# facebookresearch/nonrigid_nerf

Hardware: NVIDIA H100
Metric: rays/sec (64c+128f samples, 8x256 MLP), example_sequence training step (higher is better)
Workload: dtype f16 (tensor-core operands; f32 accumulate)

## Files before the change

### include/nrnerf_b200.h

```cpp
#ifndef NRNERF_B200_H
#define NRNERF_B200_H

#include <stddef.h>
#include <stdint.h>

#ifdef __cplusplus
extern "C" {
#endif

#define NRN_ABI_VERSION 4

#define NRN_OK 0
#define NRN_E_INVALID (-1)
#define NRN_E_CUDA (-2)
#define NRN_E_DEVICE (-3)

int nrn_abi_version(void);
const char* nrn_last_error(void);

int nrn_device_error(int* code_out);

size_t nrn_packed_nerf_bytes(void);
size_t nrn_packed_bender_bytes(void);
int nrn_pack_nerf(const float* const* w, const float* const* b, int input_ch, int out_ch, void* packed,
// ... 69 lines not shown
  const float* d_acc_map;
  float* d_raw;
  void* stream;
} NrnCompositeBwdArgs;
int nrn_composite_backward(const NrnCompositeBwdArgs* args);

size_t nrn_stash_bytes(int n_rays, int n_samples);
size_t nrn_grad_stash_bytes(int n_rays, int n_samples);
size_t nrn_relu_mask_bytes(int n_rays, int n_samples);
size_t nrn_wgrad_scratch_bytes(void);
int nrn_nerf_grad_floats(int out_ch);
int nrn_bender_grad_floats(void);
typedef struct NrnFieldBwdArgs {
  int32_t n_rays, n_samples, out_ch;
  const float* d_raw;
  const void* stash;
  void* grad_stash;
  float* wgrad_scratch;
  const void* nerf_packed;
  const void* bender_packed;
  const float* unmasked_offsets;
  const float* rigidity_mask;
  const float* d_unmasked_offsets;
  const float* d_rigidity_mask;
  int32_t use_cutoff;  float rigidity_cutoff;
  int32_t use_scaling; float scaling;
  float* nerf_grad;
  float* bender_grad;
  float* d_latents;
  void* stream;
  float* nerf_grad_head;
  int32_t accumulate_nerf, accumulate_bender;
  const void* relu_mask;
} NrnFieldBwdArgs;
int nrn_field_backward(const NrnFieldBwdArgs* args);

int nrn_tc_latent_bias(const float* latents, int64_t latent_stride, int n_rays, const float* w0, const float* b0, const float* w5,
                       const float* b5, float* ray_bias, void* stream);
int nrn_field_forward_tc(const NrnFieldArgs* args, const float* ray_bias);
int nrn_nerf_tc_grad_floats(int out_ch);

size_t nrn_packed_views_bytes(void);
int nrn_pack_views(const float* const* w, const float* const* b, void* packed, void* stream);
size_t nrn_views_workspace_bytes(int n_rays, int n_samples);
typedef struct NrnViewArgs {
  const void* views_packed;
  const float* viewdirs;
  int64_t viewdirs_stride;
  void* workspace;
} NrnViewArgs;
int nrn_field_forward_views(const NrnFieldArgs* args, const NrnViewArgs* views);
size_t nrn_packed_views_t_bytes(void);
int nrn_pack_views_t(const float* const* w, void* packed, void* stream);
size_t nrn_views_stash_bytes(int n_rays, int n_samples);
size_t nrn_views_grad_stash_bytes(int n_rays, int n_samples);
size_t nrn_hv_mask_bytes(int n_rays, int n_samples);
int nrn_nerf_views_grad_floats(void);
typedef struct NrnViewTrainArgs {
  void* views_stash;
  void* hv_mask;
} NrnViewTrainArgs;
int nrn_field_forward_views_train(const NrnFieldArgs* args, const NrnViewArgs* views, const NrnViewTrainArgs* train);
typedef struct NrnViewBwdArgs {
  const void* views_t_packed;
  const void* views_stash;
  void* views_grad_stash;
// ... 159 lines not shown
```

### nonrigid_nerf_b200/_lib.py

```python
from __future__ import annotations

import ctypes as C
import os
import threading

_HERE = os.path.dirname(os.path.abspath(__file__))
LIB_PATH = os.path.join(_HERE, "libnrnerf_b200.so")
ABI_VERSION = 4

_f32p = C.POINTER(C.c_float)
_vp = C.c_void_p


class NrnFieldArgs(C.Structure):
    _fields_ = [
        ("rays", _vp), ("z_vals", _vp), ("points", _vp), ("points_stride", C.c_int64),
        ("latents", _vp), ("latent_stride", C.c_int64),
        ("n_rays", C.c_int32), ("n_samples", C.c_int32),
        ("nerf_packed", _vp), ("bender_packed", _vp),
        ("out_ch", C.c_int32),
        ("use_cutoff", C.c_int32), ("rigidity_cutoff", C.c_float),
        ("use_scaling", C.c_int32), ("scaling", C.c_float),
        ("use_removal", C.c_int32), ("removal_threshold", C.c_float),
        ("raw", _vp), ("initial_input_pts", _vp), ("input_pts", _vp), ("unmasked_offsets", _vp),
        ("masked_offsets", _vp), ("rigidity_mask", _vp),
        ("stash", _vp),
        ("stream", _vp),
        ("relu_mask", _vp),
    ]


class NrnViewArgs(C.Structure):
    _fields_ = [
        ("views_packed", _vp), ("viewdirs", _vp), ("viewdirs_stride", C.c_int64), ("workspace", _vp),
    ]


class NrnViewTrainArgs(C.Structure):
    _fields_ = [("views_stash", _vp), ("hv_mask", _vp)]


class NrnViewBwdArgs(C.Structure):
    _fields_ = [("views_t_packed", _vp), ("views_stash", _vp), ("views_grad_stash", _vp), ("hv_mask", _vp)]


class NrnFieldBwdArgs(C.Structure):
    _fields_ = [
        ("n_rays", C.c_int32), ("n_samples", C.c_int32), ("out_ch", C.c_int32),
        ("d_raw", _vp), ("stash", _vp), ("grad_stash", _vp), ("wgrad_scratch", _vp),
        ("nerf_packed", _vp), ("bender_packed", _vp),
        ("unmasked_offsets", _vp), ("rigidity_mask", _vp), ("d_unmasked_offsets", _vp), ("d_rigidity_mask", _vp),
        ("use_cutoff", C.c_int32), ("rigidity_cutoff", C.c_float),
        ("use_scaling", C.c_int32), ("scaling", C.c_float),
        ("nerf_grad", _vp), ("bender_grad", _vp), ("d_latents", _vp),
        ("stream", _vp),
        ("nerf_grad_head", _vp), ("accumulate_nerf", C.c_int32), ("accumulate_bender", C.c_int32),
        ("relu_mask", _vp),
    ]


class NrnTcBwdArgs(C.Structure):
    _fields_ = [
        ("latents", _vp), ("latent_stride", C.c_int64), ("w0", _vp), ("w5", _vp), ("d_latents", _vp), ("workspace", _vp),
    ]


class NrnDivArgs(C.Structure):
    _fields_ = [
        ("n_rays", C.c_int32), ("n_samples", C.c_int32),
        ("relu_mask", _vp), ("e", _vp), ("unmasked_offsets", _vp), ("rigidity_mask", _vp), ("weights", _vp),
        ("weights_are_opacity_alpha", C.c_int32),
        ("bender_packed", _vp),
        ("tangent_stash", _vp), ("d", _vp), ("alpha", _vp), ("beta", _vp), ("tau_c", _vp), ("loss", _vp),
        ("G", _vp), ("g_ray", _vp), ("G_workspace", _vp), ("adjoint_stash", _vp), ("wgrad_scratch", _vp), ("d_unmasked_offsets", _vp),
        ("d_rigidity_mask", _vp), ("bender_grad", _vp),
        ("stream", _vp),
        ("accumulate_bender", C.c_int32),
    ]


class NrnRayLossArgs(C.Structure):
    _fields_ = [
        ("n_rays", C.c_int32), ("n_samples", C.c_int32),
        ("rgb", _vp), ("rgb0", _vp), ("target", _vp), ("weights", _vp), ("unmasked_offsets", _vp), ("rigidity_mask", _vp),
        ("lam_offsets", C.c_float), ("lam_rigidity", C.c_float),
        ("loss", _vp), ("u_rgb", _vp), ("u_rgb0", _vp), ("u_unmasked_offsets", _vp), ("u_rigidity_mask", _vp),
        ("stream", _vp),
        ("sched_step", _vp), ("sched_n_iters", C.c_float), ("divergence", _vp), ("lam_divergence", C.c_float), ("u_divergence", _vp),
    ]

# ... 195 lines not shown
```

### nonrigid_nerf_b200/autograd.py

```python
from __future__ import annotations

import ctypes as C
from typing import Dict, Optional, Tuple

import torch

from . import _lib, ops


def _knobs(net):
    bender = net.ray_bender[0]
    cutoff = getattr(bender, "rigidity_test_time_cutoff", None) if bender is not None else None
    scaling = getattr(bender, "test_time_scaling", None) if bender is not None else None
    removal = getattr(net, "test_time_nonrigid_object_removal_threshold", None)
    return cutoff, scaling, removal


def _tc_net(net):
    if not getattr(net, "time_conditioned_baseline", False):
        return None
    if net.ray_bender[0] is not None:
        raise RuntimeError("nonrigid_nerf_b200: the time_conditioned_baseline NeRF requires ray bending to be turned off "
                           "(ray_bender must be None)")
    return net
# ... 14 lines not shown
        for i in range(3):
            bend += [rig_w[i], rig_b[i]]
    return nerf, bend


def _split_flat(flat: torch.Tensor, like):
    out, o = [], 0
    for p in like:
        n = p.numel()
        out.append(flat[o:o + n].view_as(p))
        o += n
    assert o == flat.numel(), (o, flat.numel())
    return out


def check_held_out(held_out: Optional[torch.Tensor], n_rays: int, device) -> Optional[torch.Tensor]:
    if held_out is None:
        return None
    if not isinstance(held_out, torch.Tensor):
        raise RuntimeError("nonrigid_nerf_b200: held_out must be a tensor ([N] bool or uint8, one entry per ray)")
    if held_out.dtype not in (torch.bool, torch.uint8):
        raise RuntimeError(f"nonrigid_nerf_b200: held_out must be bool or uint8 (0/1 per ray), got {held_out.dtype}")
    if held_out.dim() != 1 or held_out.shape[0] != n_rays:
        raise RuntimeError(f"nonrigid_nerf_b200: held_out must have shape [{n_rays}] (one entry per ray), got {list(held_out.shape)}")
    if held_out.device != torch.device(device):
        raise RuntimeError(f"nonrigid_nerf_b200: held_out must be on the rays' device {device}, got {held_out.device}")
    return held_out.contiguous().view(torch.uint8)


def _zero_held_rows(d_raw: torch.Tensor, held: Optional[torch.Tensor]) -> torch.Tensor:
    if held is None:
        return d_raw
    return d_raw.masked_fill(held.view(-1, 1, 1).bool(), 0.0)


class _FieldTrainFn(torch.autograd.Function):

    @staticmethod
    def forward(ctx, net, rays, z_vals, latents, held, n_nerf, *params):
        bender = net.ray_bender[0]
        cutoff, scaling, removal = _knobs(net)
        if removal is not None:
            raise RuntimeError("nonrigid_nerf_b200: test_time_nonrigid_object_removal_threshold is a test-time knob; "
                               "it is not differentiable")
        nerf_pack = ops.pack_nerf(net)
        bender_pack = ops.pack_bender(bender) if bender is not None else None
        out_ch = net.output_linear.weight.shape[0]
        n, s = z_vals.shape
        lib = _lib.load()
        stash = torch.empty(lib.nrn_stash_bytes(n, s), dtype=torch.uint8, device=z_vals.device)
        relu_mask = torch.empty(lib.nrn_relu_mask_bytes(n, s), dtype=torch.uint8, device=z_vals.device)
        tc = _tc_net(net)
        ctx.tc_latents = None
        if tc is not None:
            ctx.tc_latents = ops.latent_rows(latents.detach(), n, z_vals.device)
            latents = ctx.tc_latents[0]
        raw, det = ops.field_forward(rays, z_vals, latents, nerf_pack, bender_pack, out_ch, cutoff, scaling, None, True, stash,
                                     relu_mask, tc)
        ctx.net, ctx.n_nerf = net, n_nerf
        ctx.shape = (n, s, out_ch)
        ctx.knobs = (cutoff, scaling)
        ctx.packs = (nerf_pack, bender_pack)
        ctx.stash = stash
        ctx.relu_mask = relu_mask
        ctx.params = params
        ctx.held = held
# ... 40 lines not shown
        nerf_grad, a.nerf_grad, a.nerf_grad_head, a.accumulate_nerf = _grad_destination(nerf_p, len(nerf_p) - 2, n_floats, dev)
        bend_grad = d_lat = None
        keep = [d_raw]
        if bender is not None:
            un, rig = ctx.saved_tensors
            a.bender_packed = bender_pack.data_ptr()
            a.unmasked_offsets, a.rigidity_mask = un.data_ptr(), rig.data_ptr()
            if d_un is not None:
                d_un = d_un.contiguous().float()
                a.d_unmasked_offsets = d_un.data_ptr()
                keep.append(d_un)
            if d_rig is not None:
                d_rig = d_rig.contiguous().float()
                a.d_rigidity_mask = d_rig.data_ptr()
                keep.append(d_rig)
            if cutoff is not None:
                a.use_cutoff, a.rigidity_cutoff = 1, float(cutoff)
            if scaling is not None:
                a.use_scaling, a.scaling = 1, float(scaling)
            bend_p = list(ctx.params[ctx.n_nerf:])
            bend_grad, a.bender_grad, _, a.accumulate_bender = _grad_destination(bend_p, len(bend_p), lib.nrn_bender_grad_floats(), dev)
            d_lat = torch.empty(n, ops.LATENT, dtype=torch.float32, device=dev)
            a.d_latents = d_lat.data_ptr()
        a.stream = torch.cuda.current_stream().cuda_stream
        if ctx.tc_latents is not None:
            lat, stride = ctx.tc_latents
            t = _lib.NrnTcBwdArgs()
            t.latents, t.latent_stride = lat.data_ptr(), stride
            t.w0, t.w5 = net.pts_linears[0].weight.data_ptr(), net.pts_linears[5].weight.data_ptr()
            d_lat = torch.empty(n, ops.LATENT, dtype=torch.float32, device=dev)
            workspace = torch.empty(lib.nrn_tc_workspace_bytes(n), dtype=torch.uint8, device=dev)
            t.d_latents, t.workspace = d_lat.data_ptr(), workspace.data_ptr()
            with torch.cuda.device(dev):
                _lib.check(lib.nrn_field_backward_tc(C.byref(a), C.byref(t)), "field_backward_tc")
        elif bender is not None and torch.are_deterministic_algorithms_enabled():
            rows = torch.empty(lib.nrn_latent_rows_bytes(n, s) // 4, dtype=torch.float32, device=dev)
            with torch.cuda.device(dev):
                if held is not None:
                    _lib.check(lib.nrn_field_backward_det_held_out(C.byref(a), rows.data_ptr(), held.data_ptr()), "field_backward_det_held_out")
                else:
                    _lib.check(lib.nrn_field_backward_det(C.byref(a), rows.data_ptr()), "field_backward_det")
        elif held is not None:
            with torch.cuda.device(dev):
                _lib.check(lib.nrn_field_backward_held_out(C.byref(a), held.data_ptr()), "field_backward_held_out")
        else:
            with torch.cuda.device(dev):
                _lib.check(lib.nrn_field_backward(C.byref(a)), "field_backward")
        grads = _param_grads(nerf_grad, nerf_p)
        if bender is not None:
            grads += _param_grads(bend_grad, bend_p)
        return (None, None, None, d_lat, None, None, *grads)


def _arena_destination(params):
    from .optim import arena_destination
    return arena_destination(list(params))


def _grad_destination(params, split: int, n_floats: int, dev):
    if all(p.requires_grad for p in params):
        dst = _arena_destination(params[:split])
        head = _arena_destination(params[split:]) if dst is not None and split < len(params) else None
        if dst is not None and (head is not None or split == len(params)):
            return None, dst, head, 1
    flat = torch.empty(n_floats, dtype=torch.float32, device=dev)
    return flat, flat.data_ptr(), None, 0


def _param_grads(flat: Optional[torch.Tensor], params):
    if flat is None:
        return [None] * len(params)
    return [g if p.requires_grad else None for g, p in zip(_split_flat(flat, params), params)]


class _LatentGatherFn(torch.autograd.Function):

    @staticmethod
    def forward(ctx, timestep, *latents):
        z = latents[0].numel()
        base, contiguous = latents[0].data_ptr(), True
# ... 85 lines not shown
        ctx.shape = (n, s)
        a = _div_args(ctx)
        a.loss = loss.data_ptr()
        if torch.are_deterministic_algorithms_enabled():
            rows = torch.empty(lib.nrn_div_loss_rows_bytes(n, s) // 4, dtype=torch.float32, device=dev)
            with torch.cuda.device(dev):
                _lib.check(lib.nrn_divergence_forward_det(C.byref(a), rows.data_ptr()), "divergence_forward_det")
        else:
            with torch.cuda.device(dev):
                _lib.check(lib.nrn_divergence_forward(C.byref(a)), "divergence_forward")
        ctx.bend_p = bend_p
        ctx.held = held
        ctx.in_shapes = (unmasked.shape, rigidity.shape)
        return loss

    @staticmethod
    def backward(ctx, g):
        n, s = ctx.shape
        dev = ctx.keep[0].device
        lib = _lib.load()
        g = g.reshape(n).contiguous().float()
        G = torch.empty(n * s, dtype=torch.float32, device=dev)
        a = _div_args(ctx)
        a.g_ray, a.G_workspace = g.data_ptr(), G.data_ptr()
        adj = torch.empty(lib.nrn_div_grad_stash_bytes(n, s), dtype=torch.uint8, device=dev)
        scratch = torch.empty(lib.nrn_wgrad_scratch_bytes(), dtype=torch.uint8, device=dev)
        d_un = torch.empty(n * s, 3, dtype=torch.float32, device=dev)
        d_rg = torch.empty(n * s, dtype=torch.float32, device=dev)
        bend_p = list(ctx.bend_p)
        bend_grad, a.bender_grad, _, a.accumulate_bender = _grad_destination(bend_p, len(bend_p), lib.nrn_bender_grad_floats(), dev)
        a.adjoint_stash, a.wgrad_scratch = adj.data_ptr(), scratch.data_ptr()
        a.d_unmasked_offsets, a.d_rigidity_mask = d_un.data_ptr(), d_rg.data_ptr()
        with torch.cuda.device(dev):
            if ctx.held is not None:
                _lib.check(lib.nrn_divergence_backward_held_out(C.byref(a), ctx.held.data_ptr()), "divergence_backward_held_out")
            else:
                _lib.check(lib.nrn_divergence_backward(C.byref(a)), "divergence_backward")
        return (d_un.view(ctx.in_shapes[0]), d_rg.view(ctx.in_shapes[1]), None, None, None, None, None, None,
                *_param_grads(bend_grad, bend_p))


def divergence_loss(unmasked: torch.Tensor, rigidity: torch.Tensor, weights: Optional[torch.Tensor], bender,
                    e: Optional[torch.Tensor] = None, opacity_alpha: Optional[torch.Tensor] = None,
                    held_out: Optional[torch.Tensor] = None) -> torch.Tensor:
    held = check_held_out(held_out, unmasked.shape[0], unmasked.device)
    relu_mask = lookup_relu_mask(unmasked)
    if relu_mask is None:
        raise RuntimeError("nonrigid_nerf_b200: no ReLU masks for these offsets -- the fused divergence term needs the "
                           "un-chunked coarse pass of the current differentiable render() call (N_rand <= chunk)")
    n, s = unmasked.shape[0], unmasked.shape[1]
    if e is None:
        e = torch.randn(n * s, 3, device=unmasked.device)
    _, bend_p = _flat_params(None, bender)
    if opacity_alpha is not None:
        return _DivergenceFn.apply(unmasked, rigidity, opacity_alpha, e, relu_mask, bender, True, held, *bend_p)
    return _DivergenceFn.apply(unmasked, rigidity, weights, e, relu_mask, bender, False, held, *bend_p)


class _RayLossFn(torch.autograd.Function):

    @staticmethod
    def forward(ctx, rgb, rgb0, target, weights, unmasked, rigidity, lam_o, lam_r, sched_step, sched_n_iters, div, lam_div):
        n = rgb.shape[0]
        dev = rgb.device
        lib = _lib.load()
        a = _lib.NrnRayLossArgs()
# ... 256 lines not shown
```

### nonrigid_nerf_b200/csrc/c_abi.cu

```cuda
#include <cstdarg>
#include <cstdio>
#include <cstring>
#include <cstdlib>
#include "../../include/nrnerf_b200.h"
#include "nrn_common.cuh"
#include "pack.cuh"
#include "ray_ops.cuh"
#include "wgrad.cuh"
#include "div.cuh"
#include "loss.cuh"
#include "adam.cuh"
#include "peer.cuh"
#include "det_reduce.cuh"
#include "eval.cuh"

namespace nrn {
cudaError_t launch_field_fwd(const FieldFwdParams& p, bool has_bender, int num_sms, cudaStream_t stream);
cudaError_t launch_field_bwd(const FieldBwdParams& p, bool has_bender, int num_sms, cudaStream_t stream);
cudaError_t launch_field_bwd_det(const FieldBwdParams& p, float* latent_rows, int num_sms, cudaStream_t stream);
cudaError_t launch_field_bwd_held(const FieldBwdParams& p, float* latent_rows, const uint8_t* held, int num_sms, cudaStream_t stream);
cudaError_t launch_field_fwd_tc(const FieldFwdParams& p, int num_sms, cudaStream_t stream);
cudaError_t launch_tc_latent_bias(const float* lat, long long lat_stride, int n_rays, const float* w0, const float* b0, const float* w5,
                                  const float* b5, float* rb, cudaStream_t stream);
cudaError_t launch_tc_latent_bwd(const TcBwdParams& p, cudaStream_t stream);
cudaError_t launch_field_bend(const FieldFwdParams& p, const ViewParams& v, int num_sms, cudaStream_t stream);
cudaError_t launch_field_views(const FieldFwdParams& p, const ViewParams& v, int num_sms, cudaStream_t stream);
cudaError_t launch_field_views_train(const FieldFwdParams& p, const ViewParams& v, const ViewTrainParams& t, int num_sms, cudaStream_t stream);
cudaError_t launch_field_bwd_views(const FieldBwdParams& p, const ViewBwdParams& v, int num_sms, cudaStream_t stream);
}

namespace {

thread_local char g_err[512] = "";

int fail(int code, const char* fmt, ...) {
  va_list ap;
  va_start(ap, fmt);
  vsnprintf(g_err, sizeof(g_err), fmt, ap);
  va_end(ap);
  return code;
}
int cuda_fail(cudaError_t e, const char* what) {
  return fail(NRN_E_CUDA, "%s: %s", what, cudaGetErrorString(e));
}

constexpr int kMaxDevices = 64;
struct DeviceState {
  int* err_word = nullptr;
  int num_sms = 0;
};
DeviceState g_dev[kMaxDevices];

int device_state(DeviceState** out) {
  int dev = 0;
  cudaError_t e = cudaGetDevice(&dev);
  if (e != cudaSuccess) return cuda_fail(e, "cudaGetDevice");
  if (dev < 0 || dev >= kMaxDevices) return fail(NRN_E_INVALID, "device index %d out of range", dev);
  DeviceState& s = g_dev[dev];
  if (!s.err_word) {
    cudaDeviceProp prop;
    e = cudaGetDeviceProperties(&prop, dev);
    if (e != cudaSuccess) return cuda_fail(e, "cudaGetDeviceProperties");
    if (prop.major != 9 || prop.minor != 0)
      return fail(NRN_E_INVALID, "nrnerf_b200 is built for sm_90a (H100) only, found sm_%d%d", prop.major, prop.minor);
    s.num_sms = prop.multiProcessorCount;
    if (const char* g = getenv("NRN_GRID")) { const int v = atoi(g); if (v > 0 && v < s.num_sms) s.num_sms = v; }
    e = cudaMalloc(&s.err_word, 4 * sizeof(int));
    if (e != cudaSuccess) return cuda_fail(e, "cudaMalloc(err word)");
    e = cudaMemset(s.err_word, 0, 4 * sizeof(int));
    if (e != cudaSuccess) return cuda_fail(e, "cudaMemset(err word)");
  }
  *out = &s;
  return NRN_OK;
}

bool aligned16(const void* p) { return (reinterpret_cast<uintptr_t>(p) & 15u) == 0; }

struct TimedLaunch {
  cudaEvent_t a, b;
  int kind;
};
bool g_timing = false;
// ... 463 lines not shown
  cudaStream_t st = static_cast<cudaStream_t>(a->stream);
  return timed(4, st, "composite_bwd_kernel", [&] { return nrn::launch_composite_bwd(p, st); });
}

size_t nrn_stash_bytes(int n_rays, int n_samples) { return static_cast<size_t>(even_tiles(n_rays, n_samples)) * nrn::kStashTileBytes; }
size_t nrn_grad_stash_bytes(int n_rays, int n_samples) { return static_cast<size_t>(even_tiles(n_rays, n_samples)) * nrn::kGradTileBytes; }
size_t nrn_relu_mask_bytes(int n_rays, int n_samples) { return static_cast<size_t>(even_tiles(n_rays, n_samples)) * nrn::kMaskTileBytes; }
size_t nrn_wgrad_scratch_bytes(void) { return static_cast<size_t>(nrn::kWgMaxCtas) * nrn::kWgScratchFloats * sizeof(float); }
int nrn_nerf_grad_floats(int out_ch) { return nrn::nerf_grad_floats(out_ch); }
int nrn_bender_grad_floats(void) { return nrn::bparam::total(); }
int nrn_nerf_tc_grad_floats(int out_ch) { return nrn::nerf_tc_grad_floats(out_ch); }
size_t nrn_tc_workspace_bytes(int n_rays) { return n_rays < 0 ? 0 : (static_cast<size_t>(n_rays) * 2 * 256 + 2 * 256 * nrn::kLatent) * sizeof(float); }

static int field_backward(const NrnFieldBwdArgs* a, const NrnTcBwdArgs* t, const char* who, float* latent_rows = nullptr,
                          const uint8_t* held = nullptr) {
  long long P;
  int tiles;
  int rc = check_field_bwd_args(a, who, &P, &tiles);
  if (rc) return rc;
  DeviceState* ds;
  rc = device_state(&ds);
  if (rc) return rc;
  if (ds->num_sms + 16 > nrn::kWgMaxCtas) return fail(NRN_E_INVALID, "%s: %d SMs exceed the scratch layout", who, ds->num_sms);
  cudaStream_t st = static_cast<cudaStream_t>(a->stream);
  const bool bend = a->bender_packed != nullptr;
  const int nerf_n = t ? nrn_nerf_tc_grad_floats(a->out_ch) : nrn_nerf_grad_floats(a->out_ch);
  const int bend_n = bend ? nrn_bender_grad_floats() : 0;
  cudaError_t e;
  if (bend && !latent_rows) {
    e = cudaMemsetAsync(a->d_latents, 0, sizeof(float) * static_cast<size_t>(a->n_rays) * nrn::kLatent, st);
    if (e != cudaSuccess) return cuda_fail(e, "memset d_latents");
  }
  if (P == 0) return zero_grads(a, nerf_n, a->out_ch * 257, bend_n, st);
  float* amax = reinterpret_cast<float*>(ds->err_word + 1);
  const nrn::FieldBwdParams p = field_bwd_params(a, P, tiles, amax, ds->err_word);
  e = nrn::launch_absmax(a->d_raw, P * a->out_ch, amax, st, false, a->out_ch, 4);
  if (e == cudaSuccess && bend && p.d_unmasked_up) e = nrn::launch_absmax(p.d_unmasked_up, P * 3, amax, st, true);
  if (e == cudaSuccess && bend && p.d_rigid_up) e = nrn::launch_absmax(p.d_rigid_up, P, amax, st, true);
  if (e != cudaSuccess) return cuda_fail(e, "absmax_kernel");
  if (held) {
    rc = timed(15, st, "field_bwd_held_kernel", [&] { return nrn::launch_field_bwd_held(p, latent_rows, held, ds->num_sms, st); });
  } else if (latent_rows) {
    rc = timed(1, st, "field_bwd_det_kernel", [&] { return nrn::launch_field_bwd_det(p, latent_rows, ds->num_sms, st); });
  } else {
    rc = timed(1, st, "field_bwd_kernel", [&] { return nrn::launch_field_bwd(p, bend, ds->num_sms, st); });
  }
  if (rc) return rc;
  if (latent_rows) {
    rc = timed(13, st, "latent_reduce_kernel", [&] { return nrn::launch_latent_reduce(latent_rows, a->d_latents, a->n_rays, a->n_samples, st); });
    if (rc) return rc;
  }
  float* dw_lat = nullptr;
  if (t) {
    nrn::TcBwdParams q{};
    q.gstash = p.gstash; q.amax = amax; q.P = P; q.S = p.S; q.n_rays = a->n_rays;
    q.latents = t->latents; q.latent_stride = t->latent_stride; q.w0 = t->w0; q.w5 = t->w5;
    q.sums = t->workspace; q.dw_lat = dw_lat = t->workspace + static_cast<size_t>(a->n_rays) * 2 * 256; q.d_latents = t->d_latents;
    rc = timed(7, st, "tc_ray_sums_kernel", [&] { return nrn::launch_tc_latent_bwd(q, st); });
    if (rc) return rc;
  }
  const nrn::WgradParams w = wgrad_params(p.stash, p.gstash, a->wgrad_scratch, amax, tiles, ds->err_word);
  const nrn::WgradDst dst{a->nerf_grad, a->nerf_grad_head, a->bender_grad, nerf_n, bend_n, a->accumulate_nerf, a->accumulate_bender};
  return timed(2, st, "wgrad_kernel", [&] { return nrn::launch_wgrad(w, bend, ds->num_sms, dst, a->out_ch, st, dw_lat); });
}

int nrn_field_backward(const NrnFieldBwdArgs* a) { return field_backward(a, nullptr, "nrn_field_backward"); }

size_t nrn_latent_rows_bytes(int n_rays, int n_samples) {
  return n_rays < 0 || n_samples < 1 ? 0 : static_cast<size_t>(n_rays) * n_samples * nrn::kLatent * sizeof(float);
}
size_t nrn_div_loss_rows_bytes(int n_rays, int n_samples) {
  return n_rays < 0 || n_samples < 1 ? 0 : static_cast<size_t>(n_rays) * n_samples * sizeof(float);
}

int nrn_field_backward_det(const NrnFieldBwdArgs* a, float* latent_rows) {
  const char* who = "nrn_field_backward_det";
  if (!a) return fail(NRN_E_INVALID, "%s: null args", who);
  if (!a->bender_packed || !a->d_latents)
    return fail(NRN_E_INVALID, "%s: needs a bender (bender_packed) and d_latents: only the bender's latent gradient has a fixed-order variant", who);
  if (a->n_rays == 0) return field_backward(a, nullptr, who);
  if (!latent_rows || !aligned16(latent_rows)) return fail(NRN_E_INVALID, "%s: null or unaligned latent_rows (nrn_latent_rows_bytes, 16-byte aligned)", who);
  return field_backward(a, nullptr, who, latent_rows);
}

static int check_held_out(const NrnFieldBwdArgs* a, const uint8_t* held, const char* who) {
  if (!a) return fail(NRN_E_INVALID, "%s: null args", who);
  if (!a->bender_packed || !a->d_latents)
    return fail(NRN_E_INVALID, "%s: needs a bender (bender_packed) and d_latents; without a bender a held-out ray contributes "
                "nothing: zero its rows of d_raw and call nrn_field_backward", who);
  if (a->n_rays > 0 && !held) return fail(NRN_E_INVALID, "%s: null held_out_rays", who);
  return NRN_OK;
}

int nrn_field_backward_held_out(const NrnFieldBwdArgs* a, const uint8_t* held_out_rays) {
  const char* who = "nrn_field_backward_held_out";
  const int rc = check_held_out(a, held_out_rays, who);
// ... 409 lines not shown
```

### nonrigid_nerf_b200/csrc/sm90_ptx.cuh

```cuda
#pragma once
#include <cuda_runtime.h>
#include <cuda_fp16.h>
#include <cuda_bf16.h>
#include <stdint.h>

namespace nrn {

__device__ __forceinline__ uint32_t smem_u32(const void* p) {
  return static_cast<uint32_t>(__cvta_generic_to_shared(p));
}

__device__ __forceinline__ void mbar_init(uint64_t* bar, uint32_t count) {
  asm volatile("mbarrier.init.shared::cta.b64 [%0], %1;\n" ::"r"(smem_u32(bar)), "r"(count) : "memory");
}
__device__ __forceinline__ void fence_mbar_init() {
  asm volatile("fence.mbarrier_init.release.cluster;\n" ::: "memory");
}
__device__ __forceinline__ void mbar_arrive(uint64_t* bar) {
  asm volatile("mbarrier.arrive.shared::cta.b64 _, [%0];\n" ::"r"(smem_u32(bar)) : "memory");
}
__device__ __forceinline__ void mbar_arrive_expect_tx(uint64_t* bar, uint32_t bytes) {
  asm volatile("mbarrier.arrive.expect_tx.shared::cta.b64 _, [%0], %1;\n" ::"r"(smem_u32(bar)), "r"(bytes)
               : "memory");
}
__device__ __forceinline__ bool mbar_try_wait(uint64_t* bar, uint32_t parity) {
  uint32_t ok;
  asm volatile(
      "{\n\t.reg .pred P;\n\t"
      "mbarrier.try_wait.parity.shared::cta.b64 P, [%1], %2;\n\t"
      "selp.b32 %0, 1, 0, P;\n\t}\n"
      : "=r"(ok)
      : "r"(smem_u32(bar)), "r"(parity)
      : "memory");
  return ok != 0;
}

__device__ __forceinline__ uint32_t cluster_ctarank() {
  uint32_t r;
  asm volatile("mov.u32 %0, %%cluster_ctarank;\n" : "=r"(r));
  return r;
}
__device__ __forceinline__ void cluster_sync() {
  asm volatile("barrier.cluster.arrive.release.aligned;\n\tbarrier.cluster.wait.acquire.aligned;\n" ::: "memory");
}
__device__ __forceinline__ uint32_t mapa_shared(const void* p, uint32_t rank) {
  uint32_t r;
// ... 329 lines not shown
```

### nonrigid_nerf_b200/csrc/wgrad.cu

```cuda
#include "nrn_common.cuh"
#include "sm90_ptx.cuh"
#include "wgrad.cuh"

namespace nrn {

namespace {

constexpr int kRingBytes = 96 * kChunkBytes;
constexpr int kMaxStages = 4;
constexpr uint32_t kPieceBytes = 16384;
constexpr int kWgThreads = 384;

struct Unit {
  int a_chunk, b_chunk;
  int dst, ld;
  int rows;
};
struct Job {
  int a_off, a_chunks;
  int b_off, b_chunks;
  int bias;
  int bias_off;
  Unit u[2];
};
// ... 156 lines not shown
            const uint4 w = *reinterpret_cast<const uint4*>(src + r * 512);
            const uint32_t wv[4] = {w.x, w.y, w.z, w.w};
#pragma unroll
            for (int qq = 0; qq < 4; ++qq) {
              t8[2 * qq] += h_lo(wv[qq]);
              t8[2 * qq + 1] += h_hi(wv[qq]);
            }
          }
        }
#pragma unroll
        for (int qq = 0; qq < 8; ++qq) s[cc * 8 + qq] = t8[qq];
      }
      bias_acc += warp_transpose_reduce(s, lane);
    }
    if constexpr (N0 > 0) {
      wgmma_wait<0>();
      acc_fence(acc0);
      acc_fence(acc1);
    }
    __syncwarp();
    if (lane == 0) {
      mbar_arrive(&sh->empty[stage]);
      if (R.paired) mbar_arrive_cluster(R.partner_empty + stage * static_cast<uint32_t>(sizeof(uint64_t)));
    }
    if (++stage == R.n_stages) { stage = 0; phase ^= 1u; }
  }
  if (!have || n_tiles_local == 0) return;
  if (jb.bias && (warp * 4 + (lane >> 3)) < jb.a_chunks) part[65536 + jb.bias_off + warp * 32 + lane] = bias_acc;
  if constexpr (N0 > 0) unit_drain(acc0, u0, part);
  if constexpr (N1 > 0) unit_drain(acc1, u1, part);
}

template <bool VIEWS>
__device__ __forceinline__ void wgrad_body(const WgradParams& p, const WgradViewParams& v) {
  extern __shared__ __align__(1024) uint8_t smem[];
  Shared* sh = reinterpret_cast<Shared*>(smem + kRingBytes);
  const int warp = threadIdx.x >> 5, lane = threadIdx.x & 31;

  int job_id = 0, split = 0, nsplit = 1, half = 0, halves = 1, part_idx = 0;
  const bool have = locate(p, blockIdx.x, job_id, split, nsplit, half, halves, part_idx);
  const Job jb = VIEWS ? views_job_desc(job_id, half, (warp >> 2) & 1) : job_desc(job_id, half, (warp >> 2) & 1, p.compact);
  const int per = (p.n_tiles + nsplit - 1) / nsplit;
  const int t_begin = have ? min(split * per, p.n_tiles) : 0;
  const int t_end = have ? min(t_begin + per, p.n_tiles) : 0;
  const int n_local = t_end - t_begin;
  const bool paired = have && halves == 2;
  const uint32_t rank = cluster_ctarank(), partner = rank ^ 1u;
  const int stage_bytes = (jb.a_chunks + jb.b_chunks) * kChunkBytes;
  const int n_stages = min(kMaxStages, kRingBytes / stage_bytes);

  if (threadIdx.x == 0) {
    for (int i = 0; i < n_stages; ++i) {
      mbar_init(&sh->full[i], 1);
      mbar_init(&sh->empty[i], paired ? 16 : 8);
    }
    sh->abort_flag = 0;
    fence_mbar_init();
  }
  cluster_sync();
  const Waiter W{&sh->abort_flag, p.err, paired, paired ? mapa_shared(&sh->abort_flag, partner) : 0u};
  const Ring R{smem, stage_bytes, n_stages, paired, paired ? mapa_shared(&sh->empty[0], partner) : 0u};

  if (warp >= 8) {
    setmaxnreg_dec<kProducerRegs>();
    if (warp == 8 && lane == 0) {
      const uint32_t a_bytes = static_cast<uint32_t>(jb.a_chunks) * kChunkBytes, b_bytes = static_cast<uint32_t>(jb.b_chunks) * kChunkBytes;
      const uint32_t b_begin = paired ? rank * (b_bytes / 2) : 0u, b_end = paired ? b_begin + b_bytes / 2 : b_bytes;
      const uint8_t* a_base = p.gstash;
      const uint8_t* b_base = p.stash;
      long long a_tile = p.gstash_tile_bytes, b_tile = p.stash_tile_bytes;
      if constexpr (VIEWS) {
        if (job_id == kJobFeature || job_id == kJobViewsF || job_id == kJobViewsE) { a_base = v.vgstash; a_tile = kVGradTileBytes; }
        if (job_id == kJobViewsF || job_id == kJobViewsE || job_id == kJobRgb) { b_base = v.vstash; b_tile = kVStashTileBytes; }
      }
      uint32_t stage = 0, phase = 0;
      for (int it = 0; it < n_local; ++it) {
        const long long tile = t_begin + it;
        const uint8_t* a_src = a_base + tile * a_tile + jb.a_off;
        const uint8_t* b_src = b_base + tile * b_tile + jb.b_off;
        W.wait(&sh->empty[stage], phase ^ 1u, 101);
        mbar_arrive_expect_tx(&sh->full[stage], a_bytes + b_bytes);
        uint8_t* dst = smem + stage * stage_bytes;
        for (uint32_t o = 0; o < a_bytes; o += kPieceBytes)
          tma_bulk_g2s(dst + o, a_src + o, a_bytes - o < kPieceBytes ? a_bytes - o : kPieceBytes, &sh->full[stage]);
        dst += a_bytes;
        for (uint32_t o = b_begin; o < b_end; o += kPieceBytes) {
          const uint32_t n = b_end - o < kPieceBytes ? b_end - o : kPieceBytes;
          if (paired) tma_bulk_g2s_multicast(dst + o, b_src + o, n, &sh->full[stage], 0x3);
          else tma_bulk_g2s(dst + o, b_src + o, n, &sh->full[stage]);
        }
        if (++stage == n_stages) { stage = 0; phase ^= 1u; }
      }
    }
  } else {
    setmaxnreg_inc<kConsumerRegs>();
    const int g = warp >> 2;
    float* part = p.scratch + static_cast<size_t>(part_idx) * kWgScratchFloats;
    const Unit& u0 = jb.u[0];
    const Unit& u1 = jb.u[1];
    if (VIEWS && job_id == kJobViewsF) {
      consume<8 * kVsF.chunks, 0>(jb, u0, u1, R, sh, W, n_local, part, have);
    } else if (VIEWS && job_id == kJobViewsE) {
      consume<8 * kVsDir.chunks, 0>(jb, u0, u1, R, sh, W, n_local, part, have);
    } else if (VIEWS && job_id == kJobRgb) {
      if (u0.rows > 0) consume<8 * kVsHv.chunks, 0>(jb, u0, u1, R, sh, W, n_local, part, have);
      else consume<0, 0>(jb, u0, u1, R, sh, W, n_local, part, have);
    } else if (VIEWS || job_id <= 9) {
      const bool mine = u0.rows > 0;
      if (job_id == 8 || job_id == 9) {
        if (mine) consume<8 * kStE.chunks, 0>(jb, u0, u1, R, sh, W, n_local, part, have);
        else consume<0, 0>(jb, u0, u1, R, sh, W, n_local, part, have);
      } else {
        if (mine) consume<8 * kHChunks, 0>(jb, u0, u1, R, sh, W, n_local, part, have);
        else consume<0, 0>(jb, u0, u1, R, sh, W, n_local, part, have);
      }
    } else if (job_id == 10) {
      if (g == 0) consume<8 * kStHb4.chunks, 8 * kStHb3.chunks>(jb, u0, u1, R, sh, W, n_local, part, have);
      else consume<8 * kStHb2.chunks, 8 * kStHb2.chunks>(jb, u0, u1, R, sh, W, n_local, part, have);
    } else {
      if (g == 0) consume<8 * kStHb1.chunks, 8 * kStHb1.chunks>(jb, u0, u1, R, sh, W, n_local, part, have);
      else consume<8 * kStBin.chunks, 8 * kStBin.chunks>(jb, u0, u1, R, sh, W, n_local, part, have);
    }
  }
  __syncwarp();
  cluster_sync();
}

}

__global__ void __launch_bounds__(kWgThreads, 1) wgrad_kernel(const WgradParams p) { wgrad_body<false>(p, WgradViewParams{}); }
__global__ void __launch_bounds__(kWgThreads, 1) wgrad_views_kernel(const WgradParams p, const WgradViewParams v) {
  wgrad_body<true>(p, v);
}


namespace {

struct Src {
  int job;
  int off;
  int off2;
  int bias;
};

__device__ __forceinline__ Src nerf_w(int job, int m, int n) { return {job, m * 256 + n, -1, 0}; }
__device__ __forceinline__ Src nerf_b(int job, int m) { return {job, m, -1, 1}; }
__device__ __forceinline__ Src bend_w(int job, int sub, int m, int n, int n2 = -1) {
  return {job, sub * 16384 + m * 128 + n, n2 >= 0 ? sub * 16384 + m * 128 + n2 : -1, 0};
}

constexpr int kLatJob = -1;
template <bool TC = false>
__device__ __forceinline__ Src nerf_src(int idx, int out_ch, bool& ok) {
  ok = true;
  constexpr int lat = TC ? kLatent : 0;
  constexpr int in0 = nerf_in(0) + lat, in5 = nerf_in(5) + lat;
  constexpr int pe = nerf_in(0);
  const int sz0 = 256 * in0 + 256, szl = 256 * 256 + 256, sz5 = 256 * in5 + 256;
// ... 156 lines not shown
  const float v = lat ? __ldg(dw_lat + s.off) : sum / scale;
  float* out;
  bool acc;
  if (idx < nerf_n) {
    const int n_pts = nerf_n - out_ch * 257;
    out = (idx >= n_pts && dst.nerf_head) ? dst.nerf_head + (idx - n_pts) : dst.nerf + idx;
    acc = dst.acc_nerf != 0;
  } else {
    out = dst.bend + (idx - nerf_n);
    acc = dst.acc_bend != 0;
  }
  *out = acc ? *out + v : v;
}


__global__ void wgrad_reduce_kernel(const WgradParams p, const WgradDst dst, int out_ch) { wgrad_reduce<false>(p, dst, out_ch, nullptr); }
__global__ void wgrad_reduce_tc_kernel(const WgradParams p, const WgradDst dst, int out_ch, const float* dw_lat) {
  wgrad_reduce<true>(p, dst, out_ch, dw_lat);
}
__global__ void wgrad_views_reduce_kernel(const WgradParams p, const WgradDst dst) {
  const int idx = blockIdx.x * blockDim.x + threadIdx.x;
  if (idx >= dst.nerf_n) return;
  const float v = split_sum(p, views_src(idx)) / loss_scale(p.amax);
  float* out = (idx >= kViewsTrunkFloats && dst.nerf_head) ? dst.nerf_head + (idx - kViewsTrunkFloats) : dst.nerf + idx;
  *out = dst.acc_nerf ? *out + v : v;
}

namespace {
constexpr int kJobCost[16] = {46, 48, 48, 48, 48, 48, 48, 48, 16 + 8 + 8, 16 + 8 + 8, 54, 24 + 18, 48, 48, 24, 20};
constexpr int job_halves(int j) { return (j >= 1 && j <= 9) || j == kJobFeature ? 2 : 1; }

template <typename... Args>
cudaError_t launch_jobs(void (*kernel)(WgradParams, Args...), int* s_max_clusters, WgradParams& p, const int* jobs, int n,
                        int num_sms, cudaStream_t st, Args... args) {
  const size_t smem = kRingBytes + sizeof(Shared) + 64;
  cudaError_t e = cudaFuncSetAttribute(kernel, cudaFuncAttributeMaxDynamicSharedMemorySize, (int)smem);
  if (e != cudaSuccess) return e;
  cudaLaunchAttribute cluster{};
  cluster.id = cudaLaunchAttributeClusterDimension;
  cluster.val.clusterDim.x = 2; cluster.val.clusterDim.y = 1; cluster.val.clusterDim.z = 1;
  cudaLaunchConfig_t cfg{};
  cfg.gridDim = dim3(2); cfg.blockDim = dim3(kWgThreads); cfg.dynamicSmemBytes = smem; cfg.stream = st;
  cfg.attrs = &cluster; cfg.numAttrs = 1;
  int dev = 0;
  e = cudaGetDevice(&dev);
  if (e != cudaSuccess) return e;
  if (dev < 0 || dev >= 64) return cudaErrorInvalidDevice;
  if (s_max_clusters[dev] <= 0) {
    e = cudaOccupancyMaxActiveClusters(&s_max_clusters[dev], kernel, &cfg);
    if (e != cudaSuccess) return e;
    if (s_max_clusters[dev] <= 0) return cudaErrorInvalidConfiguration;
  }
  const int max_ctas = min(num_sms, 2 * s_max_clusters[dev]) & ~1;

  int splits[16], halves[16], used = 0;
  for (int j = 0; j < n; ++j) {
    splits[j] = 1;
    halves[j] = job_halves(jobs[j]);
    used += halves[j];
  }
  const int tiles = p.n_tiles > 0 ? p.n_tiles : 1;
  for (;;) {
    int best = -1;
    long long best_load = -1;
    for (int j = 0; j < n; ++j) {
      const int sp = splits[j];
      if (sp >= tiles || used + halves[j] > max_ctas) continue;
      const long long load = static_cast<long long>(kJobCost[jobs[j]]) * ((tiles + sp - 1) / sp);
      if (load > best_load) { best_load = load; best = j; }
    }
    if (best < 0) break;
    ++splits[best];
    used += halves[best];
  }
  p.n_jobs = 0;
  for (int h = 2; h >= 1; --h)
    for (int j = 0; j < n; ++j)
      if (halves[j] == h) { p.job_ids[p.n_jobs] = jobs[j]; p.splits[p.n_jobs] = splits[j]; p.halves[p.n_jobs] = h; ++p.n_jobs; }
  if (p.n_tiles > 0) {
    cfg.gridDim = dim3((used + 1) & ~1);
    e = cudaLaunchKernelEx(&cfg, kernel, p, args...);
    if (e != cudaSuccess) return e;
  }
  return cudaSuccess;
}
}

cudaError_t launch_wgrad(WgradParams p, bool has_bender, int num_sms, const WgradDst& dst, int out_ch, cudaStream_t st,
                         const float* tc_dw_lat) {
  int first = 0, last = has_bender ? 12 : 10;
  if (p.compact) { first = 10; last = 12; p.stash_tile_bytes = kTanTileBytes; p.gstash_tile_bytes = kAdjTileBytes; }
  else { p.stash_tile_bytes = kStashTileBytes; p.gstash_tile_bytes = kGradTileBytes; }

  int jobs[12], n_jobs = 0;
  for (int j = first; j < last; ++j) jobs[n_jobs++] = j;
  static int s_max_clusters[64];
  cudaError_t e = launch_jobs(wgrad_kernel, s_max_clusters, p, jobs, n_jobs, num_sms, st);
  if (e != cudaSuccess) return e;
  const int n = dst.nerf_n + dst.bend_n;
  if (n > 0 && tc_dw_lat) wgrad_reduce_tc_kernel<<<(n + 255) / 256, 256, 0, st>>>(p, dst, out_ch, tc_dw_lat);
  else if (n > 0) wgrad_reduce_kernel<<<(n + 255) / 256, 256, 0, st>>>(p, dst, out_ch);
  return cudaGetLastError();
}

cudaError_t launch_wgrad_views(WgradParams p, const WgradViewParams& v, int num_sms, const WgradDst& dst, cudaStream_t st) {
  int jobs[14];
  for (int j = 0; j < 14; ++j) jobs[j] = j < 10 ? j : kJobFeature + (j - 10);
  p.stash_tile_bytes = kStashTileBytes; p.gstash_tile_bytes = kGradTileBytes;
  static int s_max_clusters[64];
  cudaError_t e = launch_jobs(wgrad_views_kernel, s_max_clusters, p, jobs, 14, num_sms, st, v);
  if (e != cudaSuccess) return e;
  if (dst.nerf_n > 0) wgrad_views_reduce_kernel<<<(dst.nerf_n + 255) / 256, 256, 0, st>>>(p, dst);
  return cudaGetLastError();
}

}
```

### nonrigid_nerf_b200/csrc/wgrad.cuh

```cuda
#pragma once
#include <cuda_runtime.h>
#include <stdint.h>

namespace nrn {

constexpr int kWgScratchFloats = 256 * 256 + 256;
constexpr int kWgMaxCtas = 192;

struct WgradParams {
  const uint8_t* stash;
  const uint8_t* gstash;
  float* scratch;
  const float* amax;
  int n_tiles;
  int compact;
  long long stash_tile_bytes, gstash_tile_bytes;
  int n_jobs;
  int job_ids[16];
  int splits[16];
  int halves[16];
  int* err;
};

struct WgradDst {
  float* nerf;
  float* nerf_head;
  float* bend;
  int nerf_n, bend_n;
  int acc_nerf, acc_bend;
};
cudaError_t launch_wgrad(WgradParams p, bool has_bender, int num_sms, const WgradDst& dst, int out_ch, cudaStream_t st,
                         const float* tc_dw_lat = nullptr);
struct WgradViewParams {
  const uint8_t* vstash;
  const uint8_t* vgstash;
};
cudaError_t launch_wgrad_views(WgradParams p, const WgradViewParams& v, int num_sms, const WgradDst& dst, cudaStream_t st);
cudaError_t launch_absmax(const float* x, long long n, float* amax, cudaStream_t st, bool accumulate = false, int row_len = 1,
                          int cols = 1);

}
```

Before: 492,500.

## Overlap field backward wgrad on side stream with next dgrad via SM partitioning

Runs the weight-gradient kernel of the field backward on a side stream so it can overlap with the next backward call's dgrad kernel. The two share the SMs through caps on CTA counts, and the wgrad kernel becomes persistent, looping over virtual CTAs with mbarrier re-init between them. The wgrad reduce step waits on an event from the pending side stream, and the amax buffer moves into scratch to avoid a shared-buffer race. The aim is to fill idle SMs across backward stages, at the cost of extra stream and event synchronisation and fewer SMs for each kernel.

```diff
diff --git a/include/nrnerf_b200.h b/include/nrnerf_b200.h
--- a/include/nrnerf_b200.h
+++ b/include/nrnerf_b200.h
@@ -125,6 +125,9 @@
   float* nerf_grad_head;
   int32_t accumulate_nerf, accumulate_bender;
   const void* relu_mask;
+  void* wgrad_stream;
+  int32_t dgrad_max_ctas, wgrad_max_ctas;
+  void* reduce_after;
 } NrnFieldBwdArgs;
 int nrn_field_backward(const NrnFieldBwdArgs* args);
 
diff --git a/nonrigid_nerf_b200/_lib.py b/nonrigid_nerf_b200/_lib.py
--- a/nonrigid_nerf_b200/_lib.py
+++ b/nonrigid_nerf_b200/_lib.py
@@ -56,6 +56,7 @@
         ("stream", _vp),
         ("nerf_grad_head", _vp), ("accumulate_nerf", C.c_int32), ("accumulate_bender", C.c_int32),
         ("relu_mask", _vp),
+        ("wgrad_stream", _vp), ("dgrad_max_ctas", C.c_int32), ("wgrad_max_ctas", C.c_int32), ("reduce_after", _vp),
     ]
 
 
diff --git a/nonrigid_nerf_b200/autograd.py b/nonrigid_nerf_b200/autograd.py
--- a/nonrigid_nerf_b200/autograd.py
+++ b/nonrigid_nerf_b200/autograd.py
@@ -70,6 +70,30 @@
     if held is None:
         return d_raw
     return d_raw.masked_fill(held.view(-1, 1, 1).bool(), 0.0)
+
+
+_OVERLAP_BACKWARD = True
+_SIDE_STREAMS = {}
+_PENDING = {}
+
+
+def _side_stream(dev) -> torch.cuda.Stream:
+    idx = torch.device(dev).index
+    if idx not in _SIDE_STREAMS:
+        _SIDE_STREAMS[idx] = torch.cuda.Stream(device=dev)
+    return _SIDE_STREAMS[idx]
+
+
+def _wait_pending(dev) -> None:
+    ev = _PENDING.get(torch.device(dev).index)
+    if ev is not None:
+        torch.cuda.current_stream(dev).wait_event(ev)
+
+
+def _overlap_caps(dev):
+    n = torch.cuda.get_device_properties(dev).multi_processor_count
+    c = max((n // 2) & ~1, 2)
+    return c, max(n - c, 1)
 
 
 class _FieldTrainFn(torch.autograd.Function):
@@ -176,20 +200,50 @@
             workspace = torch.empty(lib.nrn_tc_workspace_bytes(n), dtype=torch.uint8, device=dev)
             t.d_latents, t.workspace = d_lat.data_ptr(), workspace.data_ptr()
             with torch.cuda.device(dev):
+                _wait_pending(dev)
                 _lib.check(lib.nrn_field_backward_tc(C.byref(a), C.byref(t)), "field_backward_tc")
         elif bender is not None and torch.are_deterministic_algorithms_enabled():
             rows = torch.empty(lib.nrn_latent_rows_bytes(n, s) // 4, dtype=torch.float32, device=dev)
             with torch.cuda.device(dev):
+                _wait_pending(dev)
                 if held is not None:
                     _lib.check(lib.nrn_field_backward_det_held_out(C.byref(a), rows.data_ptr(), held.data_ptr()), "field_backward_det_held_out")
                 else:
                     _lib.check(lib.nrn_field_backward_det(C.byref(a), rows.data_ptr()), "field_backward_det")
         elif held is not None:
             with torch.cuda.device(dev):
+                _wait_pending(dev)
                 _lib.check(lib.nrn_field_backward_held_out(C.byref(a), held.data_ptr()), "field_backward_held_out")
         else:
+            overlap = _OVERLAP_BACKWARD and nerf_grad is None and bend_grad is None
+            idx = torch.device(dev).index
+            pending = _PENDING.get(idx) if overlap else None
+            side = None
+            if pending is not None:
+                a.dgrad_max_ctas = _overlap_caps(dev)[1]
+                a.reduce_after = pending.cuda_event
+            elif overlap:
+                side = _side_stream(dev)
+                a.wgrad_stream = side.cuda_stream
+                a.wgrad_max_ctas = _overlap_caps(dev)[0]
+            else:
+                _wait_pending(dev)
             with torch.cuda.device(dev):
                 _lib.check(lib.nrn_field_backward(C.byref(a)), "field_backward")
+            if side is not None:
+                for t in (ctx.stash, gstash, scratch):
+                    t.record_stream(side)
+                ev = torch.cuda.Event()
+                ev.record(side)
+                _PENDING[idx] = ev
+                main = torch.cuda.current_stream(dev)
+
+                def join():
+                    main.wait_event(ev)
+                    if _PENDING.get(idx) is ev:
+                        del _PENDING[idx]
+
+                torch.autograd.Variable._execution_engine.queue_callback(join)
         grads = _param_grads(nerf_grad, nerf_p)
         if bender is not None:
             grads += _param_grads(bend_grad, bend_p)
@@ -341,6 +395,7 @@
         a.adjoint_stash, a.wgrad_scratch = adj.data_ptr(), scratch.data_ptr()
         a.d_unmasked_offsets, a.d_rigidity_mask = d_un.data_ptr(), d_rg.data_ptr()
         with torch.cuda.device(dev):
+            _wait_pending(dev)
             if ctx.held is not None:
                 _lib.check(lib.nrn_divergence_backward_held_out(C.byref(a), ctx.held.data_ptr()), "divergence_backward_held_out")
             else:
diff --git a/nonrigid_nerf_b200/csrc/c_abi.cu b/nonrigid_nerf_b200/csrc/c_abi.cu
--- a/nonrigid_nerf_b200/csrc/c_abi.cu
+++ b/nonrigid_nerf_b200/csrc/c_abi.cu
@@ -48,6 +48,7 @@
 struct DeviceState {
   int* err_word = nullptr;
   int num_sms = 0;
+  cudaEvent_t dgrad_done = nullptr;
 };
 DeviceState g_dev[kMaxDevices];
 
@@ -577,18 +578,19 @@
     if (e != cudaSuccess) return cuda_fail(e, "memset d_latents");
   }
   if (P == 0) return zero_grads(a, nerf_n, a->out_ch * 257, bend_n, st);
-  float* amax = reinterpret_cast<float*>(ds->err_word + 1);
+  float* amax = a->wgrad_scratch + static_cast<size_t>(nrn::kWgMaxCtas - 1) * nrn::kWgScratchFloats;
+  const int dgrad_sms = a->dgrad_max_ctas > 0 && a->dgrad_max_ctas < ds->num_sms ? a->dgrad_max_ctas : ds->num_sms;
   const nrn::FieldBwdParams p = field_bwd_params(a, P, tiles, amax, ds->err_word);
   e = nrn::launch_absmax(a->d_raw, P * a->out_ch, amax, st, false, a->out_ch, 4);
   if (e == cudaSuccess && bend && p.d_unmasked_up) e = nrn::launch_absmax(p.d_unmasked_up, P * 3, amax, st, true);
   if (e == cudaSuccess && bend && p.d_rigid_up) e = nrn::launch_absmax(p.d_rigid_up, P, amax, st, true);
   if (e != cudaSuccess) return cuda_fail(e, "absmax_kernel");
   if (held) {
-    rc = timed(15, st, "field_bwd_held_kernel", [&] { return nrn::launch_field_bwd_held(p, latent_rows, held, ds->num_sms, st); });
+    rc = timed(15, st, "field_bwd_held_kernel", [&] { return nrn::launch_field_bwd_held(p, latent_rows, held, dgrad_sms, st); });
   } else if (latent_rows) {
-    rc = timed(1, st, "field_bwd_det_kernel", [&] { return nrn::launch_field_bwd_det(p, latent_rows, ds->num_sms, st); });
+    rc = timed(1, st, "field_bwd_det_kernel", [&] { return nrn::launch_field_bwd_det(p, latent_rows, dgrad_sms, st); });
   } else {
-    rc = timed(1, st, "field_bwd_kernel", [&] { return nrn::launch_field_bwd(p, bend, ds->num_sms, st); });
+    rc = timed(1, st, "field_bwd_kernel", [&] { return nrn::launch_field_bwd(p, bend, dgrad_sms, st); });
   }
   if (rc) return rc;
   if (latent_rows) {
@@ -606,7 +608,21 @@
   }
   const nrn::WgradParams w = wgrad_params(p.stash, p.gstash, a->wgrad_scratch, amax, tiles, ds->err_word);
   const nrn::WgradDst dst{a->nerf_grad, a->nerf_grad_head, a->bender_grad, nerf_n, bend_n, a->accumulate_nerf, a->accumulate_bender};
-  return timed(2, st, "wgrad_kernel", [&] { return nrn::launch_wgrad(w, bend, ds->num_sms, dst, a->out_ch, st, dw_lat); });
+  cudaStream_t wst = st;
+  if (a->wgrad_stream) {
+    wst = static_cast<cudaStream_t>(a->wgrad_stream);
+    if (!ds->dgrad_done) {
+      e = cudaEventCreateWithFlags(&ds->dgrad_done, cudaEventDisableTiming);
+      if (e != cudaSuccess) return cuda_fail(e, "cudaEventCreate");
+    }
+    e = cudaEventRecord(ds->dgrad_done, st);
+    if (e == cudaSuccess) e = cudaStreamWaitEvent(wst, ds->dgrad_done, 0);
+    if (e != cudaSuccess) return cuda_fail(e, "wgrad_stream fork");
+  }
+  return timed(2, wst, "wgrad_kernel", [&] {
+    return nrn::launch_wgrad(w, bend, ds->num_sms, dst, a->out_ch, wst, dw_lat, a->wgrad_max_ctas,
+                             static_cast<cudaEvent_t>(a->reduce_after));
+  });
 }
 
 int nrn_field_backward(const NrnFieldBwdArgs* a) { return field_backward(a, nullptr, "nrn_field_backward"); }
diff --git a/nonrigid_nerf_b200/csrc/sm90_ptx.cuh b/nonrigid_nerf_b200/csrc/sm90_ptx.cuh
--- a/nonrigid_nerf_b200/csrc/sm90_ptx.cuh
+++ b/nonrigid_nerf_b200/csrc/sm90_ptx.cuh
@@ -12,6 +12,9 @@
 
 __device__ __forceinline__ void mbar_init(uint64_t* bar, uint32_t count) {
   asm volatile("mbarrier.init.shared::cta.b64 [%0], %1;\n" ::"r"(smem_u32(bar)), "r"(count) : "memory");
+}
+__device__ __forceinline__ void mbar_inval(uint64_t* bar) {
+  asm volatile("mbarrier.inval.shared::cta.b64 [%0];\n" ::"r"(smem_u32(bar)) : "memory");
 }
 __device__ __forceinline__ void fence_mbar_init() {
   asm volatile("fence.mbarrier_init.release.cluster;\n" ::: "memory");
diff --git a/nonrigid_nerf_b200/csrc/wgrad.cu b/nonrigid_nerf_b200/csrc/wgrad.cu
--- a/nonrigid_nerf_b200/csrc/wgrad.cu
+++ b/nonrigid_nerf_b200/csrc/wgrad.cu
@@ -212,13 +212,13 @@
 }
 
 template <bool VIEWS>
-__device__ __forceinline__ void wgrad_body(const WgradParams& p, const WgradViewParams& v) {
+__device__ __forceinline__ void wgrad_vcta(const WgradParams& p, const WgradViewParams& v, int vcta) {
   extern __shared__ __align__(1024) uint8_t smem[];
   Shared* sh = reinterpret_cast<Shared*>(smem + kRingBytes);
   const int warp = threadIdx.x >> 5, lane = threadIdx.x & 31;
 
   int job_id = 0, split = 0, nsplit = 1, half = 0, halves = 1, part_idx = 0;
-  const bool have = locate(p, blockIdx.x, job_id, split, nsplit, half, halves, part_idx);
+  const bool have = locate(p, vcta, job_id, split, nsplit, half, halves, part_idx);
   const Job jb = VIEWS ? views_job_desc(job_id, half, (warp >> 2) & 1) : job_desc(job_id, half, (warp >> 2) & 1, p.compact);
   const int per = (p.n_tiles + nsplit - 1) / nsplit;
   const int t_begin = have ? min(split * per, p.n_tiles) : 0;
@@ -230,11 +230,14 @@
   const int n_stages = min(kMaxStages, kRingBytes / stage_bytes);
 
   if (threadIdx.x == 0) {
+    for (int i = 0; i < kMaxStages; ++i) {
+      mbar_inval(&sh->full[i]);
+      mbar_inval(&sh->empty[i]);
+    }
     for (int i = 0; i < n_stages; ++i) {
       mbar_init(&sh->full[i], 1);
       mbar_init(&sh->empty[i], paired ? 16 : 8);
     }
-    sh->abort_flag = 0;
     fence_mbar_init();
   }
   cluster_sync();
@@ -242,7 +245,6 @@
   const Ring R{smem, stage_bytes, n_stages, paired, paired ? mapa_shared(&sh->empty[0], partner) : 0u};
 
   if (warp >= 8) {
-    setmaxnreg_dec<kProducerRegs>();
     if (warp == 8 && lane == 0) {
       const uint32_t a_bytes = static_cast<uint32_t>(jb.a_chunks) * kChunkBytes, b_bytes = static_cast<uint32_t>(jb.b_chunks) * kChunkBytes;
       const uint32_t b_begin = paired ? rank * (b_bytes / 2) : 0u, b_end = paired ? b_begin + b_bytes / 2 : b_bytes;
@@ -273,7 +275,6 @@
       }
     }
   } else {
-    setmaxnreg_inc<kConsumerRegs>();
     const int g = warp >> 2;
     float* part = p.scratch + static_cast<size_t>(part_idx) * kWgScratchFloats;
     const Unit& u0 = jb.u[0];
@@ -304,6 +305,24 @@
   }
   __syncwarp();
   cluster_sync();
+}
+
+
+template <bool VIEWS>
+__device__ __forceinline__ void wgrad_body(const WgradParams& p, const WgradViewParams& v) {
+  extern __shared__ __align__(1024) uint8_t smem[];
+  Shared* sh = reinterpret_cast<Shared*>(smem + kRingBytes);
+  if (threadIdx.x == 0) {
+    for (int i = 0; i < kMaxStages; ++i) {
+      mbar_init(&sh->full[i], 1);
+      mbar_init(&sh->empty[i], 1);
+    }
+    sh->abort_flag = 0;
+  }
+  if ((threadIdx.x >> 5) >= 8) setmaxnreg_dec<kProducerRegs>();
+  else setmaxnreg_inc<kConsumerRegs>();
+#pragma unroll 1
+  for (int vcta = blockIdx.x; vcta < p.n_ctas; vcta += gridDim.x) wgrad_vcta<VIEWS>(p, v, vcta);
 }
 
 }
@@ -526,7 +545,7 @@
 
 template <typename... Args>
 cudaError_t launch_jobs(void (*kernel)(WgradParams, Args...), int* s_max_clusters, WgradParams& p, const int* jobs, int n,
-                        int num_sms, cudaStream_t st, Args... args) {
+                        int num_sms, int cap, cudaStream_t st, Args... args) {
   const size_t smem = kRingBytes + sizeof(Shared) + 64;
   cudaError_t e = cudaFuncSetAttribute(kernel, cudaFuncAttributeMaxDynamicSharedMemorySize, (int)smem);
   if (e != cudaSuccess) return e;
@@ -571,8 +590,9 @@
   for (int h = 2; h >= 1; --h)
     for (int j = 0; j < n; ++j)
       if (halves[j] == h) { p.job_ids[p.n_jobs] = jobs[j]; p.splits[p.n_jobs] = splits[j]; p.halves[p.n_jobs] = h; ++p.n_jobs; }
+  p.n_ctas = (used + 1) & ~1;
   if (p.n_tiles > 0) {
-    cfg.gridDim = dim3((used + 1) & ~1);
+    cfg.gridDim = dim3(cap > 0 && cap < p.n_ctas ? max(cap & ~1, 2) : p.n_ctas);
     e = cudaLaunchKernelEx(&cfg, kernel, p, args...);
     if (e != cudaSuccess) return e;
   }
@@ -581,7 +601,7 @@
 }
 
 cudaError_t launch_wgrad(WgradParams p, bool has_bender, int num_sms, const WgradDst& dst, int out_ch, cudaStream_t st,
-                         const float* tc_dw_lat) {
+                         const float* tc_dw_lat, int max_ctas, cudaEvent_t reduce_after) {
   int first = 0, last = has_bender ? 12 : 10;
   if (p.compact) { first = 10; last = 12; p.stash_tile_bytes = kTanTileBytes; p.gstash_tile_bytes = kAdjTileBytes; }
   else { p.stash_tile_bytes = kStashTileBytes; p.gstash_tile_bytes = kGradTileBytes; }
@@ -589,8 +609,12 @@
   int jobs[12], n_jobs = 0;
   for (int j = first; j < last; ++j) jobs[n_jobs++] = j;
   static int s_max_clusters[64];
-  cudaError_t e = launch_jobs(wgrad_kernel, s_max_clusters, p, jobs, n_jobs, num_sms, st);
+  cudaError_t e = launch_jobs(wgrad_kernel, s_max_clusters, p, jobs, n_jobs, num_sms, max_ctas, st);
   if (e != cudaSuccess) return e;
+  if (reduce_after) {
+    e = cudaStreamWaitEvent(st, reduce_after, 0);
+    if (e != cudaSuccess) return e;
+  }
   const int n = dst.nerf_n + dst.bend_n;
   if (n > 0 && tc_dw_lat) wgrad_reduce_tc_kernel<<<(n + 255) / 256, 256, 0, st>>>(p, dst, out_ch, tc_dw_lat);
   else if (n > 0) wgrad_reduce_kernel<<<(n + 255) / 256, 256, 0, st>>>(p, dst, out_ch);
@@ -602,7 +626,7 @@
   for (int j = 0; j < 14; ++j) jobs[j] = j < 10 ? j : kJobFeature + (j - 10);
   p.stash_tile_bytes = kStashTileBytes; p.gstash_tile_bytes = kGradTileBytes;
   static int s_max_clusters[64];
-  cudaError_t e = launch_jobs(wgrad_views_kernel, s_max_clusters, p, jobs, 14, num_sms, st, v);
+  cudaError_t e = launch_jobs(wgrad_views_kernel, s_max_clusters, p, jobs, 14, num_sms, 0, st, v);
   if (e != cudaSuccess) return e;
   if (dst.nerf_n > 0) wgrad_views_reduce_kernel<<<(dst.nerf_n + 255) / 256, 256, 0, st>>>(p, dst);
   return cudaGetLastError();
diff --git a/nonrigid_nerf_b200/csrc/wgrad.cuh b/nonrigid_nerf_b200/csrc/wgrad.cuh
--- a/nonrigid_nerf_b200/csrc/wgrad.cuh
+++ b/nonrigid_nerf_b200/csrc/wgrad.cuh
@@ -19,6 +19,7 @@
   int job_ids[16];
   int splits[16];
   int halves[16];
+  int n_ctas;
   int* err;
 };
 
@@ -30,7 +31,7 @@
   int acc_nerf, acc_bend;
 };
 cudaError_t launch_wgrad(WgradParams p, bool has_bender, int num_sms, const WgradDst& dst, int out_ch, cudaStream_t st,
-                         const float* tc_dw_lat = nullptr);
+                         const float* tc_dw_lat = nullptr, int max_ctas = 0, cudaEvent_t reduce_after = nullptr);
 struct WgradViewParams {
   const uint8_t* vstash;
   const uint8_t* vgstash;
```

New measurement: 500,000 (median of 6 runs). 1.02x the previous value.
